# paramhanji/sin-inn

Hardware: AMD Instinct MI355X
Metric: training frames/sec at 256x256 bs=16 (higher is better)
Workload: dtype f32; 1 GPU; BASELINE configs[1]: 8-block INN (SRF, -c 4 x 2 levels), 256x256x3, fp32, synthetic clip (64 frames, lr_window 10), batch 16/GPU, full training step (fwd+bwd, rev+bwd, Adam); height=256, width=256, global_batch=16, num_coupling=4, architecture=SRF, parallelism=dp1, hip_graph=False

## Files before the change

### sin-inn_amd/csrc/conv_mfma.hip

```cpp
#include "conv_mfma_impl.h"

namespace sininn {

int conv_dispatch_k3(ConvDev& d, hipStream_t st, int force_cfg);
int conv_dispatch_k1(ConvDev& d, hipStream_t st, int force_cfg);
int conv32_dispatch_k3(ConvDev& d, hipStream_t st, int force_cfg, bool must);
int conv32_dispatch_k1(ConvDev& d, hipStream_t st, int force_cfg, bool must);
int wino_dispatch_k3(ConvDev& d, hipStream_t st, int cg2);

int g_conv_dma = 0;
static int g_force_cfg = 0;
static int g_force_ck = 0;
static int g_ablate = 0;

int conv_bf16_launch(const sininn_conv_args* a, hipStream_t st);

int conv_prepare(const sininn_conv_args* a, ConvDev& d) {
  SININN_CHECK(a != nullptr, "conv: null args");
  SININN_CHECK(a->ksize == 1 || a->ksize == 3, "conv: ksize %d not in {1,3}", a->ksize);
  SININN_CHECK(a->Cin > 0 && a->Cin % 8 == 0, "conv: Cin=%d must be a positive multiple of 8", a->Cin);
  SININN_CHECK(a->Np > 0 && a->Np % 16 == 0, "conv: Np=%d must be a positive multiple of 16", a->Np);
  SININN_CHECK(a->B > 0 && a->H > 0 && a->W > 0, "conv: bad image shape %dx%dx%d", a->B, a->H, a->W);
  SININN_CHECK((long)a->B * a->H * a->W * (long)(a->in_stride > a->out_stride ? a->in_stride : a->out_stride) < (1l << 31),
               "conv: tensor too large for 32-bit pixel offsets");
  SININN_CHECK(a->in && a->w && a->out, "conv: null tensor pointer");
  SININN_CHECK((a->in_stride >= a->Cin || a->in_group_stride > 0) && a->in_stride % 4 == 0 && aligned16(a->in),
               "conv: input must be 16-byte aligned with stride %% 4 == 0 (stride=%d)", a->in_stride);
  SININN_CHECK(aligned16(a->w), "conv: packed weights must be 16-byte aligned");
  const bool couple = a->mode == SININN_CONV_COUPLE_FWD || a->mode == SININN_CONV_COUPLE_INV;
  if (couple) {
    SININN_CHECK(a->Co > 0 && a->Co % 8 == 0 && a->Np == 2 * a->Co, "conv: coupling needs Np == 2*Co, Co %% 8 == 0 (Np=%d Co=%d)", a->Np, a->Co);
    SININN_CHECK(a->v != nullptr && a->v_stride >= a->Co, "conv: coupling needs v");
    SININN_CHECK(a->clamp > 0.f, "conv: clamp must be > 0");
    SININN_CHECK(a->out_stride >= a->Co, "conv: out_stride < Co");
  } else {
    SININN_CHECK(a->N > 0 && a->N <= a->Np && (a->out_stride >= a->N || a->out_group_stride > 0), "conv: bad N=%d (Np=%d, out_stride=%d)", a->N, a->Np, a->out_stride);
    if (a->mode == SININN_CONV_RELU) SININN_CHECK(a->bias != nullptr, "conv: RELU mode needs bias");
    if (a->mode == SININN_CONV_MASK) SININN_CHECK(a->mask != nullptr && (a->mask_stride >= a->N || a->mask_group_stride > 0), "conv: MASK mode needs mask");
    const bool cbwd = a->mode == SININN_CONV_ADD_CBWD_FWD || a->mode == SININN_CONV_ADD_CBWD_INV;
    if (a->mode == SININN_CONV_ADD || cbwd) SININN_CHECK(a->addend != nullptr, "conv: ADD mode needs addend");
    if (cbwd) SININN_CHECK(a->v && a->sbuf && a->out2 && a->Co == a->N && a->out_stride >= 2 * a->Co && a->clamp > 0.f, "conv: ADD_CBWD needs v, sbuf, out2, Co == N, out_stride >= 2*Co");
    if ((a->mode == SININN_CONV_LINEAR || a->mode == SININN_CONV_ADD) && a->mask)
      SININN_CHECK(a->Co >= 0 && a->Co % 4 == 0 && a->mask_stride >= a->N && a->mask_stride % 4 == 0 && aligned16(a->mask) && a->mask_group_stride <= 0,
                   "conv: LeakyReLU tail needs Co %% 4 == 0 and a 16-byte aligned pixel-major mask (Co=%d, mask_stride=%d)", a->Co, a->mask_stride);
    if (a->mode == SININN_CONV_IRN_FWD || a->mode == SININN_CONV_IRN_INV)
      SININN_CHECK(a->mask && a->v && a->mask_stride >= a->N && a->v_stride >= a->N && a->clamp > 0.f, "conv: IRN modes need aux (mask), v and clamp");
  }
  SININN_CHECK(aligned16(a->out) && a->out_stride % 4 == 0, "conv: out must be 16-byte aligned with stride %% 4 == 0");
  SININN_CHECK(!a->bias || aligned16(a->bias), "conv: bias must be 16-byte aligned");
  if (couple) {
    SININN_CHECK(aligned16(a->v) && a->v_stride % 4 == 0, "conv: v must be 16-byte aligned with stride %% 4 == 0");
    SININN_CHECK(!a->out2 || (aligned16(a->out2) && a->out2_stride % 4 == 0), "conv: out2 must be 16-byte aligned");
    SININN_CHECK(!a->sbuf || aligned16(a->sbuf), "conv: sbuf must be 16-byte aligned");
  }
  if (a->mode == SININN_CONV_MASK) SININN_CHECK(aligned16(a->mask) && a->mask_stride % 4 == 0, "conv: mask must be 16-byte aligned");
  SININN_CHECK(a->N % 4 == 0 || couple, "conv: N must be a multiple of 4");
  if ((a->mode == SININN_CONV_ADD || a->mode == SININN_CONV_ADD_CBWD_FWD || a->mode == SININN_CONV_ADD_CBWD_INV) && !a->addend_map)
    SININN_CHECK(aligned16(a->addend) && a->addend_stride % 4 == 0, "conv: addend must be 16-byte aligned");
  d.in = a->in; d.in_stride = a->in_stride; d.Cin = a->Cin;
  d.w = a->w; d.bias = a->bias; d.Np = a->Np;
  d.B = a->B; d.H = a->H; d.W = a->W;
  d.out = a->out; d.out_stride = a->out_stride; d.N = a->N; d.out_map = a->out_map;
  d.v = a->v; d.v_stride = a->v_stride; d.out2 = a->out2; d.out2_stride = a->out2_stride;
  d.sbuf = a->sbuf; d.logdet = a->logdet; d.Co = a->Co; d.clamp = a->clamp;
  d.mask = a->mask; d.mask_stride = a->mask_stride;
  d.addend = a->addend; d.addend_stride = a->addend_stride; d.addend_map = a->addend_map;
  d.mode = a->mode;
  d.col_tile = a->col_tile;
  d.stamp = a->stamp;
  d.ablate = g_ablate;
  d.in_chunk = a->in_group_stride > 0 ? a->in_group_stride : 8;
  d.out_gs = a->out_group_stride > 0 ? (size_t)a->out_group_stride : 0;
  d.mask_gs = a->mask_group_stride > 0 ? (size_t)a->mask_group_stride : 0;
  if (d.out_gs || d.mask_gs) {
    SININN_CHECK(a->winograd && (a->mode == SININN_CONV_RELU || a->mode == SININN_CONV_MASK) && a->N % 64 == 0 && a->N == a->Np,
                 "conv: channel-group-major out / mask needs a Winograd RELU / MASK conv with N == Np, N %% 64 == 0");
    SININN_CHECK(!d.mask_gs || a->mode == SININN_CONV_MASK, "conv: mask_group_stride without MASK mode");
  }
  if (a->in_group_stride > 0) SININN_CHECK(a->winograd && a->in_stride == 8, "conv: the channel-group-major input layout needs the Winograd kernels and in_stride == 8");
  if (a->winograd) {
    SININN_CHECK((unsigned long long)a->H * a->W * a->in_stride * 4ull < (1ull << 31),
                 "conv: one image of the input (%d x %d x stride %d floats) exceeds the 2 GB a Winograd block addresses", a->H, a->W, a->in_stride);
    SININN_CHECK((unsigned long long)(a->Cin / 8) * (unsigned long long)d.in_chunk * 4ull < (1ull << 32), "conv: input channel-group stride too large");
  }
  SININN_CHECK(a->mode >= 0 && a->mode <= SININN_CONV_ADD_CBWD_INV, "conv: unknown mode %d", a->mode);
  int ck = 8;
  for (int c : {32, 24, 16, 8}) if (a->Cin % c == 0) { ck = c; break; }
  if (g_force_ck && a->Cin % g_force_ck == 0 && g_force_ck % 8 == 0 && g_force_ck <= 32) ck = g_force_ck;
  d.CK = ck;
  d.tiles_x = d.tiles_y = 0;
  return 0;
}

int conv_launch(const sininn_conv_args* a, hipStream_t st) {
  SININN_CHECK(a != nullptr, "conv: null args");
  if (a->w_bf16) return conv_bf16_launch(a, st);
  ConvDev d;
  if (int rc = conv_prepare(a, d)) return rc;
  const bool couple = a->mode == SININN_CONV_COUPLE_FWD || a->mode == SININN_CONV_COUPLE_INV;
  if (a->winograd) {
    SININN_CHECK(a->ksize == 3, "conv: the Winograd pack needs ksize 3");
    d.col_tile = (couple && a->col_tile == 32) ? 32 : 16;
    if (couple && d.col_tile == 32) SININN_CHECK(a->Co % 16 == 0, "conv: col_tile 32 needs Co %% 16 == 0");
    return wino_dispatch_k3(d, st, g_force_cfg % 16);
  }
  const int tile = couple ? (a->col_tile == 32 ? 32 : 16) : ((a->Np % 32 == 0 && g_force_cfg < 10) ? 32 : 16);
  if (couple && tile == 32) SININN_CHECK(a->Co % 16 == 0, "conv: col_tile 32 needs Co %% 16 == 0 (Co=%d)", a->Co);
  const int fc = g_force_cfg % 10;
  if (tile == 32) {
    const int rc = (a->ksize == 3) ? conv32_dispatch_k3(d, st, fc, couple) : conv32_dispatch_k1(d, st, fc, couple);
    if (rc >= 0) return rc;
  }
  if (a->ksize == 3) return conv_dispatch_k3(d, st, fc);
  return conv_dispatch_k1(d, st, fc);
}

void conv_set_test_hooks(int force_cfg, int force_ck) {
  g_force_cfg = force_cfg % 100; g_force_ck = force_ck; g_ablate = force_cfg / 1000;
  const int dma = (force_cfg / 100) % 10;
  if (dma) g_conv_dma = (dma == 1);
}

}
```

### sin-inn_amd/csrc/conv_mfma_k3.hip

```cpp
#include "conv32_impl.h"
#include "wino_impl.h"
namespace sininn {
int conv_dispatch_k3(ConvDev& d, hipStream_t st, int force_cfg) { return dispatch<3>(d, st, force_cfg); }
int wino_dispatch_k3(ConvDev& d, hipStream_t st, int cg2) { return wino_dispatch(d, st, cg2); }
int conv32_dispatch_k3(ConvDev& d, hipStream_t st, int force_cfg, bool must) { return dispatch32<3>(d, st, force_cfg, must); }
}
```

Baseline: 1965 frames/s.

## Add small-Cin Winograd kernel keeping the whole input tile resident in LDS

Adds a specialized Winograd F(2x2,3x3) conv kernel for Cin 24 or 48 with Np=256 in RELU/MASK modes. It loads all input channel chunks for a 16x16 output tile into LDS once, then loops over four 64-column output passes while double-buffering the transformed weights. The goal is to stop re-reading and re-transforming input across output-channel groups and to cut launches for these small-K first-layer convs. In exchange it runs one block per CU with 512 threads and heavy LDS use, which limits occupancy, and it adds a new code path that must match the existing epilogue.

```diff
diff --git a/sin-inn_amd/csrc/conv_mfma.hip b/sin-inn_amd/csrc/conv_mfma.hip
--- a/sin-inn_amd/csrc/conv_mfma.hip
+++ b/sin-inn_amd/csrc/conv_mfma.hip
@@ -7,6 +7,8 @@
 int conv32_dispatch_k3(ConvDev& d, hipStream_t st, int force_cfg, bool must);
 int conv32_dispatch_k1(ConvDev& d, hipStream_t st, int force_cfg, bool must);
 int wino_dispatch_k3(ConvDev& d, hipStream_t st, int cg2);
+bool wino_smallk_supported_k3(const ConvDev& d);
+int wino_smallk_launch_k3(ConvDev& d, hipStream_t st);
 
 int g_conv_dma = 0;
 static int g_force_cfg = 0;
@@ -102,6 +104,7 @@
     SININN_CHECK(a->ksize == 3, "conv: the Winograd pack needs ksize 3");
     d.col_tile = (couple && a->col_tile == 32) ? 32 : 16;
     if (couple && d.col_tile == 32) SININN_CHECK(a->Co % 16 == 0, "conv: col_tile 32 needs Co %% 16 == 0");
+    if (!(g_force_cfg & 16) && wino_smallk_supported_k3(d)) return wino_smallk_launch_k3(d, st);
     return wino_dispatch_k3(d, st, g_force_cfg % 16);
   }
   const int tile = couple ? (a->col_tile == 32 ? 32 : 16) : ((a->Np % 32 == 0 && g_force_cfg < 10) ? 32 : 16);
diff --git a/sin-inn_amd/csrc/conv_mfma_k3.hip b/sin-inn_amd/csrc/conv_mfma_k3.hip
--- a/sin-inn_amd/csrc/conv_mfma_k3.hip
+++ b/sin-inn_amd/csrc/conv_mfma_k3.hip
@@ -1,7 +1,10 @@
 #include "conv32_impl.h"
 #include "wino_impl.h"
+#include "wino_smallk_impl.h"
 namespace sininn {
 int conv_dispatch_k3(ConvDev& d, hipStream_t st, int force_cfg) { return dispatch<3>(d, st, force_cfg); }
 int wino_dispatch_k3(ConvDev& d, hipStream_t st, int cg2) { return wino_dispatch(d, st, cg2); }
+bool wino_smallk_supported_k3(const ConvDev& d) { return wino_smallk_supported(d); }
+int wino_smallk_launch_k3(ConvDev& d, hipStream_t st) { return wino_smallk_launch(d, st); }
 int conv32_dispatch_k3(ConvDev& d, hipStream_t st, int force_cfg, bool must) { return dispatch32<3>(d, st, force_cfg, must); }
 }
diff --git a/sin-inn_amd/csrc/wino_smallk_impl.h b/sin-inn_amd/csrc/wino_smallk_impl.h
--- /dev/null
+++ b/sin-inn_amd/csrc/wino_smallk_impl.h
@@ -0,0 +1,241 @@
+#pragma once
+#include "wino_impl.h"
+
+namespace sininn {
+
+constexpr int WSK_BN = 64, WSK_NP = 256, WSK_NTHR = 512;
+constexpr int WSK_IN_BUF = 18 * (18 * 12 + 4) + 4;
+constexpr int WSK_U_BUF = 16 * WSK_BN * 12;
+
+template <int NCH>
+__global__ __launch_bounds__(WSK_NTHR, 1) void wino_smallk_kernel(ConvDev p) {
+  constexpr int CK = 8, NT = 2;
+  constexpr int NTHR = WSK_NTHR;
+  constexpr int IW = 18, NPIX_IN = 18 * 18;
+  constexpr int BG = NT * 16, BN = WSK_BN, NPASS = WSK_NP / BN;
+  constexpr int SI = 12, SU = 12;
+  constexpr int PITCH = IW * SI + 4;
+  constexpr int IN_BUF = WSK_IN_BUF;
+  constexpr int IN_Q = NPIX_IN * 2;
+  constexpr int IN_F4 = (IN_Q * NCH + NTHR - 1) / NTHR;
+  constexpr int U_F4 = (16 * BN * 2) / NTHR;
+  constexpr int NSTEP = NPASS * NCH;
+  static_assert((16 * BN * 2) % NTHR == 0, "every thread slot of the U staging loop is a real quad");
+
+  extern __shared__ __attribute__((aligned(16))) float smem[];
+  float* const in_lds = smem;
+  float* const u_lds = smem + NCH * IN_BUF;
+
+  const int tid = threadIdx.x;
+  stamp_begin(p);
+  const int wave = (tid >> 6) & 3, grp = tid >> 8, lane = tid & 63;
+  const int li = lane & 15, kq = lane >> 4;
+
+  int bid = blockIdx.x;
+  const int tx = bid % p.tiles_x; bid /= p.tiles_x;
+  const int ty = bid % p.tiles_y;
+  const int b = bid / p.tiles_y;
+  const int y0 = ty * 16, x0 = tx * 16;
+
+  const __amdgpu_buffer_rsrc_t in_rs = buf_rsrc(p.in + (size_t)b * p.H * p.W * p.in_stride), u_rs = buf_rsrc(p.w);
+  const unsigned in_step = (unsigned)p.in_chunk * 4u;
+  constexpr unsigned u_step = (unsigned)(WSK_NP * CK) * 4u, u_pass = (unsigned)(BN * CK) * 4u;
+
+  {
+    f32x4 in_reg[IN_F4];
+    int in_loff[IN_F4];
+#pragma unroll
+    for (int r = 0; r < IN_F4; ++r) {
+      const int f = tid + NTHR * r;
+      const int chunk = f / IN_Q, g = f - chunk * IN_Q;
+      const int pix = g >> 1, c4 = g & 1;
+      const int py = pix / IW, px = pix - py * IW;
+      const int gy = y0 + py - 1, gx = x0 + px - 1;
+      const bool inside = chunk < NCH;
+      const bool inimg = inside && gy >= 0 && gy < p.H && gx >= 0 && gx < p.W;
+      in_loff[r] = inside ? (chunk * IN_BUF + py * PITCH + ((py >> 1) & 1) * 4 + px * SI + c4 * 4) : -1;
+      in_reg[r] = buf_load4(in_rs, inimg ? (unsigned)(((gy * p.W + gx) * p.in_stride + c4 * 4) * 4) + (unsigned)chunk * in_step : BUF_OOB, 0u);
+    }
+#pragma unroll
+    for (int r = 0; r < IN_F4; ++r)
+      if (in_loff[r] >= 0) *reinterpret_cast<f32x4*>(in_lds + in_loff[r]) = in_reg[r];
+  }
+
+  const int u_c4 = tid & 1, u_col = (tid >> 1) % BN, u_pos0 = (tid >> 1) / BN;
+  const int u_loff0 = (u_pos0 * BN + u_col) * SU + u_c4 * 4;
+  const unsigned u_goff0 = (unsigned)(((u_pos0 * NCH * WSK_NP + u_col) * CK + u_c4 * 4) * 4);
+  constexpr int U_LSTEP = (NTHR / 2 / BN) * BN * SU;
+  constexpr unsigned U_GSTEP = (unsigned)((NTHR / 2 / BN) * NCH * WSK_NP * CK * 4);
+  f32x4 u_reg[U_F4];
+  auto load_u = [&](int step) {
+    const int pass = step / NCH, chunk = step - pass * NCH;
+    const unsigned so = (unsigned)chunk * u_step + (unsigned)pass * u_pass;
+#pragma unroll
+    for (int r = 0; r < U_F4; ++r) u_reg[r] = buf_load4(u_rs, u_goff0 + (unsigned)r * U_GSTEP, so);
+  };
+  auto store_u = [&]() {
+#pragma unroll
+    for (int r = 0; r < U_F4; ++r) *reinterpret_cast<f32x4*>(u_lds + u_loff0 + r * U_LSTEP) = u_reg[r];
+  };
+
+  load_u(0);
+  store_u();
+  load_u(1);
+  __syncthreads();
+
+  const int a_ty = 2 * wave + (li >> 3), a_tx = li & 7;
+  const int a_base01 = (2 * a_ty) * PITCH + (a_ty & 1) * 4 + (2 * a_tx) * SI + 2 * kq;
+  const int a_base23 = (2 * a_ty) * PITCH + ((a_ty + 1) & 1) * 4 + (2 * a_tx) * SI + 2 * kq;
+  const unsigned Uc = lds_addr(u_lds + (grp * BG + li) * SU + 2 * kq);
+  __shared__ float red[NTHR / 64];
+
+#pragma unroll 1
+  for (int pass = 0; pass < NPASS; ++pass) {
+    f32x4 acc[16][NT];
+#pragma unroll
+    for (int q = 0; q < 16; ++q)
+#pragma unroll
+      for (int n = 0; n < NT; ++n) acc[q][n] = (f32x4){0.f, 0.f, 0.f, 0.f};
+
+#pragma unroll 1
+    for (int it = 0; it < NCH; ++it) {
+      const unsigned A01 = lds_addr(in_lds + it * IN_BUF + a_base01);
+      const unsigned A23 = lds_addr(in_lds + it * IN_BUF + a_base23);
+
+      f32x2 v[4][4];
+      {
+        f32x2 d[4][4];
+        static_for<0, 16>([&](auto i) {
+          constexpr int a = decltype(i)::value >> 2, c = decltype(i)::value & 3;
+          d[a][c] = lds_read_b64<(a * PITCH + c * SI) * 4>(a < 2 ? A01 : A23);
+        });
+        asm volatile("s_waitcnt lgkmcnt(0)"
+                     : "+v"(d[0][0]), "+v"(d[0][1]), "+v"(d[0][2]), "+v"(d[0][3]), "+v"(d[1][0]), "+v"(d[1][1]), "+v"(d[1][2]),
+                       "+v"(d[1][3]), "+v"(d[2][0]), "+v"(d[2][1]), "+v"(d[2][2]), "+v"(d[2][3]), "+v"(d[3][0]), "+v"(d[3][1]),
+                       "+v"(d[3][2]), "+v"(d[3][3]));
+        f32x2 t[4][4];
+#pragma unroll
+        for (int c = 0; c < 4; ++c) {
+          t[0][c] = d[0][c] - d[2][c];
+          t[1][c] = d[1][c] + d[2][c];
+          t[2][c] = d[2][c] - d[1][c];
+          t[3][c] = d[1][c] - d[3][c];
+        }
+#pragma unroll
+        for (int a = 0; a < 4; ++a) {
+          v[a][0] = t[a][0] - t[a][2];
+          v[a][1] = t[a][1] + t[a][2];
+          v[a][2] = t[a][2] - t[a][1];
+          v[a][3] = t[a][1] - t[a][3];
+        }
+      }
+      constexpr int PF = 2;
+      f32x2 bf[PF + 1][NT];
+      static_for<0, PF>([&](auto qq) {
+        constexpr int q = decltype(qq)::value;
+        bf[q][0] = lds_read_b64<((q * BN) * SU) * 4>(Uc);
+        bf[q][1] = lds_read_b64<((q * BN + 16) * SU) * 4>(Uc);
+      });
+      static_for<0, 16>([&](auto qq) {
+        constexpr int q = decltype(qq)::value;
+        if constexpr (q + PF < 16) {
+          bf[(q + PF) % (PF + 1)][0] = lds_read_b64<(((q + PF) * BN) * SU) * 4>(Uc);
+          bf[(q + PF) % (PF + 1)][1] = lds_read_b64<(((q + PF) * BN + 16) * SU) * 4>(Uc);
+        }
+        constexpr int newer = (q + PF < 16 ? PF : 15 - q) * 2;
+        lds_wait<newer>(bf[q % (PF + 1)][0], bf[q % (PF + 1)][1]);
+        acc[q][0] = __builtin_amdgcn_mfma_f32_16x16x4f32(v[q >> 2][q & 3].x, bf[q % (PF + 1)][0].x, acc[q][0], 0, 0, 0);
+        acc[q][1] = __builtin_amdgcn_mfma_f32_16x16x4f32(v[q >> 2][q & 3].x, bf[q % (PF + 1)][1].x, acc[q][1], 0, 0, 0);
+        acc[q][0] = __builtin_amdgcn_mfma_f32_16x16x4f32(v[q >> 2][q & 3].y, bf[q % (PF + 1)][0].y, acc[q][0], 0, 0, 0);
+        acc[q][1] = __builtin_amdgcn_mfma_f32_16x16x4f32(v[q >> 2][q & 3].y, bf[q % (PF + 1)][1].y, acc[q][1], 0, 0, 0);
+      });
+      __syncthreads();
+      if (it + 1 < NCH) {
+        const int step = pass * NCH + it;
+        store_u();
+        if (step + 2 < NSTEP) load_u(step + 2);
+        __syncthreads();
+      }
+    }
+
+    constexpr int TS = BN + 4;
+    float* const T = u_lds;
+    float yv[NT][4][4];
+#pragma unroll
+    for (int n = 0; n < NT; ++n)
+#pragma unroll
+      for (int r = 0; r < 4; ++r) {
+        float m[16];
+#pragma unroll
+        for (int q = 0; q < 16; ++q) m[q] = acc[q][n][r];
+        float r0[4], r1[4];
+#pragma unroll
+        for (int c = 0; c < 4; ++c) {
+          r0[c] = m[0 * 4 + c] + m[1 * 4 + c] + m[2 * 4 + c];
+          r1[c] = m[1 * 4 + c] - m[2 * 4 + c] - m[3 * 4 + c];
+        }
+        yv[n][r][0] = r0[0] + r0[1] + r0[2];
+        yv[n][r][1] = r0[1] - r0[2] - r0[3];
+        yv[n][r][2] = r1[0] + r1[1] + r1[2];
+        yv[n][r][3] = r1[1] - r1[2] - r1[3];
+      }
+#pragma unroll 1
+    for (int half = 0; half < 2; ++half) {
+      if ((wave >> 1) == half) {
+#pragma unroll
+        for (int n = 0; n < NT; ++n)
+#pragma unroll
+          for (int r = 0; r < 4; ++r) {
+            const int tl = 4 * kq + r;
+            const int oy = 2 * (2 * (wave & 1) + (tl >> 3)), ox = 2 * (tl & 7);
+            float* t00 = T + (oy * 16 + ox) * TS + grp * BG + n * 16 + li;
+            t00[0] = yv[n][r][0];
+            t00[TS] = yv[n][r][1];
+            t00[16 * TS] = yv[n][r][2];
+            t00[17 * TS] = yv[n][r][3];
+          }
+      }
+      __syncthreads();
+      conv_epilogue_tile<8, BN, 8, NTHR>(p, T, b, y0 + 8 * half, x0, pass * BN, tid, red);
+      __syncthreads();
+    }
+    if (pass + 1 < NPASS) {
+      const int step = pass * NCH + NCH - 1;
+      store_u();
+      if (step + 2 < NSTEP) load_u(step + 2);
+      __syncthreads();
+    }
+  }
+  stamp_end(p);
+}
+
+constexpr size_t wino_smallk_lds(int nch) { return (size_t)(nch * WSK_IN_BUF + WSK_U_BUF) * sizeof(float); }
+
+template <int NCH>
+static int wino_smallk_launch_n(ConvDev& d, hipStream_t st) {
+  constexpr size_t lds = wino_smallk_lds(NCH);
+  static_assert(lds + 64 <= 160 * 1024, "LDS tile too large");
+  static_assert((size_t)128 * (WSK_BN + 4) * sizeof(float) <= (size_t)WSK_U_BUF * sizeof(float), "half T must fit the U buffer");
+  d.tiles_x = d.W / 16;
+  d.tiles_y = d.H / 16;
+  auto k = wino_smallk_kernel<NCH>;
+  hipError_t e = hipFuncSetAttribute(reinterpret_cast<const void*>(k), hipFuncAttributeMaxDynamicSharedMemorySize, (int)lds);
+  if (e != hipSuccess) { set_error("wino_smallk: cannot raise LDS limit to %zu", lds); return 1; }
+  hipLaunchKernelGGL(k, dim3(d.tiles_x * d.tiles_y * d.B), dim3(WSK_NTHR), lds, st, d);
+  SININN_LAUNCH_CHECK("wino_smallk");
+  return 0;
+}
+
+static bool wino_smallk_supported(const ConvDev& d) {
+  if (d.Np != WSK_NP || !(d.Cin == 24 || d.Cin == 48)) return false;
+  if (d.mode != SININN_CONV_RELU && d.mode != SININN_CONV_MASK) return false;
+  if (d.H % 16 != 0 || d.W % 16 != 0) return false;
+  const unsigned long long last = (unsigned long long)d.H * d.W * d.in_stride * 4ull + (unsigned long long)(d.Cin / 8 - 1) * d.in_chunk * 4ull;
+  return last < (1ull << 31);
+}
+
+static int wino_smallk_launch(ConvDev& d, hipStream_t st) {
+  return d.Cin == 24 ? wino_smallk_launch_n<3>(d, st) : wino_smallk_launch_n<6>(d, st);
+}
+
+}
```

Result: no change. 1954 frames/s (-0.6%).
